# aymenboudhina/Multimodal_VQVAE_compression_audio_tactile

Measured on AMD Instinct MI355X. Metric: encode+VQ+decode token-frames/sec (1 frame = 13.33 ms of paired 24 kHz audio+tactile), higher is better.
Workload: dtype f32

## Files before the change

multimodal_vqvae_compression_audio_tactile_amd/csrc/conv1d_mfma.hpp:

```cpp
#pragma once
#include <hip/hip_runtime.h>
#include <stdio.h>
#include <stdlib.h>
#include <type_traits>
#include "det_math.hpp"
#include "kernels_small.hpp"

namespace mvq {

struct ConvArgs;
inline bool conv_dma_rows_ok(const ConvArgs& a);

__device__ __attribute__((aligned(16))) static const float g_zero16[4] = {0.0f, 0.0f, 0.0f, 0.0f};

int prof_begin(const char* kernel_name, double flops, hipStream_t s);
void prof_end(int idx, hipStream_t s);
bool prof_enabled();

typedef float f32x16 __attribute__((ext_vector_type(16)));
typedef float f32x4 __attribute__((ext_vector_type(4)));

struct ConvArgs {
    const float* x;
    const float* wp;
    const float* bias;
    const float* alpha_in;
    const float* residual;
    const float* alpha_out;
    float* y;
    int B, Cin, Tin, Cout, Tout;
    int pad;
    int Mpad;
    int Mrows;
    int Ncols;
    int n_tiles;
    int n_base;
    int n_tiles_max;
    int row_fast;
    int act;
    int dma;
    int up_s, up_p;
    int vec4;
    int ovec4;
    const float* alpha_mid;
    const float* w2p;
    const float* bias2;
    float* y2;
    const float* alpha2;
    const float* dsn_src;
    const float* dsn_alpha;
    int tvalid;
    int tper, tper_valid;
    unsigned tper_magic;
    int up_per_out, up_valid_out, up_seg, up_btrue;
    unsigned up_magic;
    int vp_seg, vp_per_in, vp_valid_in, vp_tin_phys, vp_btrue, vp_per_out, vp_valid_out;
    unsigned vp_magic_in, vp_magic_out;
    char* name_out;
    int name_len;
};

typedef float f32x16_t __attribute__((ext_vector_type(16)));

template <int OFF>
__device__ __forceinline__ float lds_read_imm(unsigned addr)
{
    static_assert(OFF >= 0 && OFF < 65536, "ds_read immediate offset is 16 bits");
    float v;
    asm volatile("ds_read_b32 %0, %1 offset:%2" : "=v"(v) : "v"(addr), "i"(OFF) : "memory");
    return v;
}
template <int P> __device__ __forceinline__ void lgkm_wait_tie(float& a, float& b)
{ asm volatile("s_waitcnt lgkmcnt(%2)" : "+v"(a), "+v"(b) : "n"(P) : "memory"); }
template <int P> __device__ __forceinline__ void lgkm_wait_tie(float& a, float& b, float& c)
{ asm volatile("s_waitcnt lgkmcnt(%3)" : "+v"(a), "+v"(b), "+v"(c) : "n"(P) : "memory"); }
template <int P> __device__ __forceinline__ void lgkm_wait_tie(float& a, float& b, float& c, float& d)
{ asm volatile("s_waitcnt lgkmcnt(%4)" : "+v"(a), "+v"(b), "+v"(c), "+v"(d) : "n"(P) : "memory"); }
template <int P> __device__ __forceinline__ void lgkm_wait_tie(float& a, float& b, float& c, float& d, float& e)
{ asm volatile("s_waitcnt lgkmcnt(%5)" : "+v"(a), "+v"(b), "+v"(c), "+v"(d), "+v"(e) : "n"(P) : "memory"); }
template <int P> __device__ __forceinline__ void lgkm_wait_tie(float& a, float& b, float& c, float& d, float& e, float& f)
{ asm volatile("s_waitcnt lgkmcnt(%6)" : "+v"(a), "+v"(b), "+v"(c), "+v"(d), "+v"(e), "+v"(f) : "n"(P) : "memory"); }
template <int P, int MT, int NT>
__device__ __forceinline__ void lgkm_wait_step(float (&av)[MT], float (&bv)[NT])
{
    static_assert(MT >= 1 && NT >= 1 && MT + NT <= 6, "operand registers per k-step");
    if constexpr (MT == 1 && NT == 1) lgkm_wait_tie<P>(av[0], bv[0]);
    else if constexpr (MT == 2 && NT == 1) lgkm_wait_tie<P>(av[0], av[1], bv[0]);
    else if constexpr (MT == 1 && NT == 2) lgkm_wait_tie<P>(av[0], bv[0], bv[1]);
    else if constexpr (MT == 2 && NT == 2) lgkm_wait_tie<P>(av[0], av[1], bv[0], bv[1]);
    else if constexpr (MT == 3 && NT == 1) lgkm_wait_tie<P>(av[0], av[1], av[2], bv[0]);
    else if constexpr (MT == 1 && NT == 3) lgkm_wait_tie<P>(av[0], bv[0], bv[1], bv[2]);
    else if constexpr (MT == 4 && NT == 1) lgkm_wait_tie<P>(av[0], av[1], av[2], av[3], bv[0]);
    else if constexpr (MT == 1 && NT == 4) lgkm_wait_tie<P>(av[0], bv[0], bv[1], bv[2], bv[3]);
    else if constexpr (MT == 3 && NT == 2) lgkm_wait_tie<P>(av[0], av[1], av[2], bv[0], bv[1]);
    else if constexpr (MT == 2 && NT == 3) lgkm_wait_tie<P>(av[0], av[1], bv[0], bv[1], bv[2]);
    else if constexpr (MT == 4 && NT == 2) lgkm_wait_tie<P>(av[0], av[1], av[2], av[3], bv[0], bv[1]);
    else if constexpr (MT == 2 && NT == 4) lgkm_wait_tie<P>(av[0], av[1], bv[0], bv[1], bv[2], bv[3]);
    else if constexpr (MT == 3 && NT == 3) lgkm_wait_tie<P>(av[0], av[1], av[2], bv[0], bv[1], bv[2]);
    else static_assert(MT + NT <= 5 || MT == 4 || NT == 4 || (MT == 3 && NT == 3), "unsupported operand shape");
}

#define MVQ_DMA_FIRST(i) "s_nop 0\n\tglobal_load_lds_dwordx4 %" #i ", off\n\t"
#define MVQ_DMA_NEXT(i) "s_add_u32 m0, m0, %[inc]\n\t" MVQ_DMA_FIRST(i)
#define MVQ_DMA_HEAD "s_mov_b32 %0, m0\n\ts_mov_b32 m0, %[dst]\n\t"
#define MVQ_DMA_TAIL "s_mov_b32 m0, %0"
template <int N, int INC>
__device__ __forceinline__ void lds_dma_burst(const float* const* src, unsigned dst)
{
    static_assert(N >= 1 && N <= 8, "pieces per burst");
    unsigned keep;
    if constexpr (N == 1)
        asm volatile(MVQ_DMA_HEAD MVQ_DMA_FIRST(1) MVQ_DMA_TAIL : "=&s"(keep) : "v"(src[0]), [dst] "s"(dst), [inc] "n"(INC) : "memory", "scc");
    else if constexpr (N == 2)
        asm volatile(MVQ_DMA_HEAD MVQ_DMA_FIRST(1) MVQ_DMA_NEXT(2) MVQ_DMA_TAIL
                     : "=&s"(keep) : "v"(src[0]), "v"(src[1]), [dst] "s"(dst), [inc] "n"(INC) : "memory", "scc");
    else if constexpr (N == 3)
        asm volatile(MVQ_DMA_HEAD MVQ_DMA_FIRST(1) MVQ_DMA_NEXT(2) MVQ_DMA_NEXT(3) MVQ_DMA_TAIL
                     : "=&s"(keep) : "v"(src[0]), "v"(src[1]), "v"(src[2]), [dst] "s"(dst), [inc] "n"(INC) : "memory", "scc");
    else if constexpr (N == 4)
        asm volatile(MVQ_DMA_HEAD MVQ_DMA_FIRST(1) MVQ_DMA_NEXT(2) MVQ_DMA_NEXT(3) MVQ_DMA_NEXT(4) MVQ_DMA_TAIL
                     : "=&s"(keep) : "v"(src[0]), "v"(src[1]), "v"(src[2]), "v"(src[3]), [dst] "s"(dst), [inc] "n"(INC) : "memory", "scc");
    else if constexpr (N == 5)
        asm volatile(MVQ_DMA_HEAD MVQ_DMA_FIRST(1) MVQ_DMA_NEXT(2) MVQ_DMA_NEXT(3) MVQ_DMA_NEXT(4) MVQ_DMA_NEXT(5) MVQ_DMA_TAIL
                     : "=&s"(keep) : "v"(src[0]), "v"(src[1]), "v"(src[2]), "v"(src[3]), "v"(src[4]), [dst] "s"(dst), [inc] "n"(INC) : "memory", "scc");
    else if constexpr (N == 6)
        asm volatile(MVQ_DMA_HEAD MVQ_DMA_FIRST(1) MVQ_DMA_NEXT(2) MVQ_DMA_NEXT(3) MVQ_DMA_NEXT(4) MVQ_DMA_NEXT(5) MVQ_DMA_NEXT(6) MVQ_DMA_TAIL
                     : "=&s"(keep) : "v"(src[0]), "v"(src[1]), "v"(src[2]), "v"(src[3]), "v"(src[4]), "v"(src[5]), [dst] "s"(dst), [inc] "n"(INC) : "memory", "scc");
    else if constexpr (N == 7)
        asm volatile(MVQ_DMA_HEAD MVQ_DMA_FIRST(1) MVQ_DMA_NEXT(2) MVQ_DMA_NEXT(3) MVQ_DMA_NEXT(4) MVQ_DMA_NEXT(5) MVQ_DMA_NEXT(6) MVQ_DMA_NEXT(7) MVQ_DMA_TAIL
                     : "=&s"(keep) : "v"(src[0]), "v"(src[1]), "v"(src[2]), "v"(src[3]), "v"(src[4]), "v"(src[5]), "v"(src[6]), [dst] "s"(dst), [inc] "n"(INC) : "memory", "scc");
    else
        asm volatile(MVQ_DMA_HEAD MVQ_DMA_FIRST(1) MVQ_DMA_NEXT(2) MVQ_DMA_NEXT(3) MVQ_DMA_NEXT(4) MVQ_DMA_NEXT(5) MVQ_DMA_NEXT(6) MVQ_DMA_NEXT(7) MVQ_DMA_NEXT(8) MVQ_DMA_TAIL
                     : "=&s"(keep) : "v"(src[0]), "v"(src[1]), "v"(src[2]), "v"(src[3]), "v"(src[4]), "v"(src[5]), "v"(src[6]), "v"(src[7]), [dst] "s"(dst), [inc] "n"(INC) : "memory", "scc");
}

template <int KS, int STRIDE, int DIL, int BM, int XP, int MT, int NT, int NS>
struct AsmOperandLoop {
    template <int S, int I>
    static __device__ __forceinline__ void load_a(float (&av)[MT], unsigned a_addr)
    {
        if constexpr (I < MT) {
            av[I] = lds_read_imm<(2 * S * BM + I * 32) * 4>(a_addr);
            load_a<S, I + 1>(av, a_addr);
        }
    }
    template <int S, int J>
    static __device__ __forceinline__ void load_b(float (&bv)[NT], unsigned b_same, unsigned b_cross)
    {
        if constexpr (J < NT) {
            constexpr int k0 = 2 * S;
            constexpr int off0 = (k0 / KS) * XP + (k0 % KS) * DIL;
            constexpr bool cross = ((k0 + 1) / KS) != (k0 / KS);
            bv[J] = lds_read_imm<(off0 + J * 32 * STRIDE) * 4>(cross ? b_cross : b_same);
            load_b<S, J + 1>(bv, b_same, b_cross);
        }
    }
    template <int S>
    static __device__ __forceinline__ void load_step(float (&av)[MT], float (&bv)[NT], unsigned a_addr, unsigned b_same, unsigned b_cross)
    {
        load_a<S, 0>(av, a_addr);
        load_b<S, 0>(bv, b_same, b_cross);
    }
    static __device__ __forceinline__ void mfma_step(f32x16_t (&acc)[MT][NT], const float (&av)[MT], const float (&bv)[NT])
    {
#pragma unroll
        for (int i = 0; i < MT; ++i)
#pragma unroll
            for (int j = 0; j < NT; ++j)
                acc[i][j] = __builtin_amdgcn_mfma_f32_32x32x2f32(av[i], bv[j], acc[i][j], 0, 0, 0);
    }
    template <int S>
    static __device__ __forceinline__ void run_from(f32x16_t (&acc)[MT][NT], float (&av0)[MT], float (&bv0)[NT], float (&av1)[MT],
                                                    float (&bv1)[NT], unsigned a_addr, unsigned b_same, unsigned b_cross)
    {
        if constexpr (S < NS) {
            if constexpr (S + 1 < NS) {
                if constexpr ((S + 1) % 2 == 0) load_step<S + 1>(av0, bv0, a_addr, b_same, b_cross);
                else load_step<S + 1>(av1, bv1, a_addr, b_same, b_cross);
            }
            constexpr int PW = (S + 1 < NS) ? MT + NT : 0;
            __builtin_amdgcn_sched_barrier(0);
            if constexpr (S % 2 == 0) lgkm_wait_step<PW, MT, NT>(av0, bv0);
            else lgkm_wait_step<PW, MT, NT>(av1, bv1);
            __builtin_amdgcn_sched_barrier(0);
            if constexpr (S % 2 == 0) mfma_step(acc, av0, bv0);
            else mfma_step(acc, av1, bv1);
            __builtin_amdgcn_sched_barrier(0);
            run_from<S + 1>(acc, av0, bv0, av1, bv1, a_addr, b_same, b_cross);
        }
    }
};

constexpr int cgcd(int a, int b) { return b == 0 ? a : cgcd(b, a % b); }

template <int KS, int STRIDE, int DIL, int CK, int MT, int NT, int WAVES_M, int WAVES_N, int UPS>
struct ConvCfg {
    static constexpr int BM = 32 * MT * WAVES_M;
    static constexpr int BN = 32 * NT * WAVES_N;
    static constexpr int KC = CK * KS;
    static constexpr int XT = (BN - 1) * STRIDE + (KS - 1) * DIL + 1;
    static constexpr bool XALIGNED = (KS == 1 && STRIDE == 1);
    static constexpr int XV = XALIGNED ? (XT + 3) / 4 : (XT + 3 + 3) / 4;
    static constexpr int XTP = XV * 4 + 4;
    static constexpr int W_FLOATS = KC * BM;
    static constexpr int X_FLOATS = CK * XTP;
    static constexpr int STAGE_FLOATS = 2 * (W_FLOATS + X_FLOATS);
    static constexpr int BNP = BN + 4;
    static constexpr int CT_FLOATS = BM * BNP;
    static constexpr int EH = ((UPS == 0 || 32 % (UPS ? UPS : 1) == 0) && MT % 2 == 0 && CT_FLOATS > STAGE_FLOATS) ? 2 : 1;
    static constexpr int CTH_FLOATS = CT_FLOATS / EH;
    static constexpr int QPR = BN / 4;
    static constexpr int CQ = cgcd(QPR, 64 * WAVES_M * WAVES_N);
    static constexpr int JN = QPR / CQ;
    static constexpr int RSTEP = (64 * WAVES_M * WAVES_N) / CQ;
    static constexpr bool REG_GEOM = (UPS == 0) && (32 % RSTEP == 0);
    static constexpr int TB_FLOATS = REG_GEOM ? 2 * BM : 0;
    static constexpr int EPI_FLOATS = CTH_FLOATS + TB_FLOATS;
    static constexpr int EPI_FLOATS_FUSE = CT_FLOATS + TB_FLOATS;
    static constexpr int LDS_FLOATS = STAGE_FLOATS > EPI_FLOATS ? STAGE_FLOATS : EPI_FLOATS;
    static constexpr bool FOUR_WAVES = WAVES_M * WAVES_N == 4;
    static constexpr bool RING_FITS = (size_t)3 * (KC * BM + CK * XV * 4) * 4 <= 64 * 1024;
    static constexpr int MIN_WPE = (FOUR_WAVES && LDS_FLOATS * 4 <= 53 * 1024 && !(WAVES_N == 4 && NT == 2) && RING_FITS && MT * NT <= 4) ? 3
                                                                                                                : (WAVES_M * WAVES_N) / 2;
    static constexpr int LDS_FLOATS_FUSE = STAGE_FLOATS > EPI_FLOATS_FUSE ? STAGE_FLOATS : EPI_FLOATS_FUSE;
    static constexpr int MIN_WPE_FUSE = (FOUR_WAVES && (LDS_FLOATS_FUSE + 5 * BM) * 4 * 3 <= 160 * 1024) ? 3 : (WAVES_M * WAVES_N) / 2;
    static constexpr int XV4 = XV * 4;
    static constexpr int DMA_STAGE_FLOATS = W_FLOATS + CK * XV4;
    static constexpr int DMA_NV = DMA_STAGE_FLOATS / 4;
    static constexpr int DMA_NU = (DMA_NV + 64 * WAVES_M * WAVES_N - 1) / (64 * WAVES_M * WAVES_N);
    static constexpr int LDS_FLOATS_DMA = 3 * DMA_STAGE_FLOATS > EPI_FLOATS ? 3 * DMA_STAGE_FLOATS : EPI_FLOATS;
    static constexpr int LDS_FLOATS_FUSE_DMA = 3 * DMA_STAGE_FLOATS > EPI_FLOATS_FUSE ? 3 * DMA_STAGE_FLOATS : EPI_FLOATS_FUSE;
    static constexpr int W_VEC = W_FLOATS / 4;
    static constexpr int NTHR = 64 * WAVES_M * WAVES_N;
    static constexpr int W_PER_THREAD = (W_VEC + NTHR - 1) / NTHR;
    static constexpr int XV_TOTAL = CK * XV;
    static constexpr int XV_PER_THREAD = (XV_TOTAL + NTHR - 1) / NTHR;
    static constexpr int XS_TOTAL = CK * XT;
    static constexpr int XS_PER_THREAD = (XS_TOTAL + NTHR - 1) / NTHR;
    static constexpr int XREGS = (4 * XV_PER_THREAD > XS_PER_THREAD) ? 4 * XV_PER_THREAD : XS_PER_THREAD;
    static_assert(WAVES_M * WAVES_N == 4 || WAVES_M * WAVES_N == 8, "block is 4 or 8 waves");
    static_assert(KC % 2 == 0, "chunk K must be even (32x32x2 MFMA)");
    static_assert(BM % 4 == 0, "float4 weight staging");
};

template <int KS, int STRIDE, int DIL, int CK, int MT, int NT, int WAVES_M, int WAVES_N, int UPS, bool VEC>
struct ConvTile {
    using C = ConvCfg<KS, STRIDE, DIL, CK, MT, NT, WAVES_M, WAVES_N, UPS>;
    const float* wp; const float* xb; const float* Al;
    float* Ws; float* Xs;
    int tid, Tin, Cin, Mpad, m0, t_in0, g_al;
    bool snake_in;

    __device__ __forceinline__ void load_chunk(int chunk, f32x4 (&wreg)[C::W_PER_THREAD], f32x4 (&xv)[C::XV_PER_THREAD], float (&xs)[C::XS_PER_THREAD]) const
    {
        const int ci0 = chunk * CK;
        const float* wsrc = wp + (size_t)ci0 * KS * Mpad + m0;
#pragma unroll
        for (int u = 0; u < C::W_PER_THREAD; ++u) {
            int v = tid + u * C::NTHR;
            if (C::W_VEC % C::NTHR != 0) v = v < C::W_VEC ? v : C::W_VEC - 1;
            const int row = v / (C::BM / 4);
            const int c4 = v - row * (C::BM / 4);
            wreg[u] = *reinterpret_cast<const f32x4*>(wsrc + (size_t)row * Mpad + c4 * 4);
        }
        if (VEC) {
#pragma unroll
            for (int u = 0; u < C::XV_PER_THREAD; ++u) {
                int e = tid + u * C::NTHR;
                if (C::XV_TOTAL % C::NTHR != 0) e = e < C::XV_TOTAL ? e : C::XV_TOTAL - 1;
                const int cl = e / C::XV;
                const int v = e - cl * C::XV;
                const int g = g_al + 4 * v;
                const bool ok = g >= 0 && g < Tin;
                const int gc = ok ? g : 0;
                xv[u] = *reinterpret_cast<const f32x4*>(xb + (size_t)(ci0 + cl) * Tin + gc);
            }
        } else {
#pragma unroll
            for (int u = 0; u < C::XS_PER_THREAD; ++u) {
                int e = tid + u * C::NTHR;
                if (C::XS_TOTAL % C::NTHR != 0) e = e < C::XS_TOTAL ? e : C::XS_TOTAL - 1;
                const int cl = e / C::XT;
                const int xi = e - cl * C::XT;
                const int g = t_in0 + xi;
                const bool ok = g >= 0 && g < Tin;
                const int gc = ok ? g : 0;
                xs[u] = xb[(size_t)(ci0 + cl) * Tin + gc];
            }
        }
    }

    __device__ __forceinline__ void store_chunk(int chunk, int buf, const f32x4 (&wreg)[C::W_PER_THREAD],
                                                const f32x4 (&xv)[C::XV_PER_THREAD],
                                                const float (&xs)[C::XS_PER_THREAD]) const
    {
        const int ci0 = chunk * CK;
        float* wdst = Ws + buf * C::W_FLOATS;
        float* xdst = Xs + buf * C::X_FLOATS;
#pragma unroll
        for (int u = 0; u < C::W_PER_THREAD; ++u) {
            const int v = tid + u * C::NTHR;
            if (C::W_VEC % C::NTHR == 0 || v < C::W_VEC) *reinterpret_cast<f32x4*>(wdst + v * 4) = wreg[u];
        }
        if (VEC) {
#pragma unroll
            for (int u = 0; u < C::XV_PER_THREAD; ++u) {
                const int e = tid + u * C::NTHR;
                const int ec = (C::XV_TOTAL % C::NTHR != 0 && e >= C::XV_TOTAL) ? C::XV_TOTAL - 1 : e;
                const int cl = ec / C::XV;
                const int v = ec - cl * C::XV;
                const int g = g_al + 4 * v;
                const bool ok = g >= 0 && g < Tin;
                f32x4 q = xv[u];
                if (!ok) q = f32x4{0.0f, 0.0f, 0.0f, 0.0f};
                if (snake_in) {
                    const float al = Al[ci0 + cl], inv = Al[Cin + ci0 + cl];
                    q.x = det_snake(q.x, al, inv); q.y = det_snake(q.y, al, inv);
                    q.z = det_snake(q.z, al, inv); q.w = det_snake(q.w, al, inv);
                }
                if (C::XV_TOTAL % C::NTHR == 0 || e < C::XV_TOTAL)
                    *reinterpret_cast<f32x4*>(xdst + cl * C::XTP + 4 * v) = q;
            }
        } else {
#pragma unroll
            for (int u = 0; u < C::XS_PER_THREAD; ++u) {
                const int e = tid + u * C::NTHR;
                const int ec = (C::XS_TOTAL % C::NTHR != 0 && e >= C::XS_TOTAL) ? C::XS_TOTAL - 1 : e;
                const int cl = ec / C::XT;
                const int xi = ec - cl * C::XT;
                const int g = t_in0 + xi;
                float q = (g >= 0 && g < Tin) ? xs[u] : 0.0f;
                if (snake_in) q = det_snake(q, Al[ci0 + cl], Al[Cin + ci0 + cl]);
                if (C::XS_TOTAL % C::NTHR == 0 || e < C::XS_TOTAL) xdst[cl * C::XTP + xi] = q;
            }
        }
    }
};

template <int KS, int STRIDE, int DIL, int CK, int MT, int NT, int WAVES_M, int WAVES_N, int UPS, bool VEC, bool FUSE>
__device__ __forceinline__ void conv1d_mfma_body(const ConvArgs& a)
{
    using C = ConvCfg<KS, STRIDE, DIL, CK, MT, NT, WAVES_M, WAVES_N, UPS>;
    extern __shared__ __attribute__((aligned(16))) float smem[];
    float* const Ws = smem;
    float* const Xs = smem + 2 * C::W_FLOATS;
    float* const Ep = smem + (FUSE ? (a.dma ? C::LDS_FLOATS_FUSE_DMA : C::LDS_FLOATS_FUSE) : (a.dma ? C::LDS_FLOATS_DMA : C::LDS_FLOATS));
    constexpr int EP_MID = 2;
    float* const Al = Ep + 3 * C::BM;

    const int tid = threadIdx.x;
    const int lane = tid & 63;
    const int wave = tid >> 6;
    const int wm = wave / WAVES_N;
    const int wn = wave % WAVES_N;
    const int l31 = lane & 31;
    const int h = lane >> 5;

    int bx = blockIdx.x, by = blockIdx.y;
    if (a.row_fast) {
        const int xcd = bx & 7, j = bx >> 3;
        by = j % a.row_fast;
        bx = (j / a.row_fast) * 8 + xcd;
        if (bx >= a.n_tiles * a.B) return;
    }
    const int b = bx / a.n_tiles;
    const int tile_n = bx - b * a.n_tiles;
    const int n0 = a.n_base + tile_n * C::BN;
    const int m0 = by * C::BM;
    const int t_in0 = n0 * STRIDE - a.pad;
    const int g_al = t_in0 & ~3;
    const int shift = VEC ? (t_in0 - g_al) : 0;
    const int Cin = a.Cin;
    const int n_chunks = Cin / CK;
    const bool snake_in = a.alpha_in != nullptr;

    if (snake_in) {
        for (int c = tid; c < Cin; c += C::NTHR) {
            const float al = a.alpha_in[c];
            Al[c] = al;
            Al[Cin + c] = 1.0f / (al + 1e-9f);
        }
    }
    for (int r = tid; r < C::BM; r += C::NTHR) {
        int m = m0 + r;
        m = m < a.Mrows ? m : a.Mrows - 1;
        const int ch = m / (UPS ? UPS : 1);
        const float* tabs[4] = {a.alpha_out, a.y2 ? a.alpha2 : nullptr, FUSE ? a.alpha_mid : (a.dsn_src ? a.dsn_alpha : nullptr), nullptr};
#pragma unroll
        for (int k = 0; k < 3; ++k) {
            Ep[k * C::BM + r] = tabs[k] ? 1.0f / (tabs[k][ch] + 1e-9f) : 1.0f;
        }
    }

    ConvTile<KS, STRIDE, DIL, CK, MT, NT, WAVES_M, WAVES_N, UPS, VEC> tile;
    tile.wp = a.wp; tile.xb = a.x + (size_t)b * Cin * a.Tin; tile.Al = Al; tile.Ws = Ws; tile.Xs = Xs;
    tile.tid = tid; tile.Tin = a.Tin; tile.Cin = Cin; tile.Mpad = a.Mpad; tile.m0 = m0; tile.t_in0 = t_in0;
    tile.g_al = g_al; tile.snake_in = snake_in;

    f32x16 acc[MT][NT];
#pragma unroll
    for (int i = 0; i < MT; ++i)
#pragma unroll
        for (int j = 0; j < NT; ++j)
#pragma unroll
            for (int r = 0; r < 16; ++r) acc[i][j][r] = 0.0f;

    f32x4 wreg[C::W_PER_THREAD];
    f32x4 xv[C::XV_PER_THREAD];
    float xs[C::XS_PER_THREAD];

    constexpr int D_SAME = DIL;
    constexpr int D_CROSS = C::XTP - (KS - 1) * DIL;
    const int a_base = h * C::BM + wm * (MT * 32) + l31;
    const int b_base = (wn * (NT * 32) + l31) * STRIDE + shift;
    const int b_same = b_base + h * D_SAME;
    const int b_cross = b_base + h * D_CROSS;

    constexpr int NS = C::KC / 2;
    auto mfma_chunk = [&](int buf) __attribute__((always_inline)) {
        const float* wsrc = Ws + buf * C::W_FLOATS + a_base;
        const float* xs_same = Xs + buf * C::X_FLOATS + b_same;
        const float* xs_cross = Xs + buf * C::X_FLOATS + b_cross;
        float av[2][MT], bv[2][NT];
        auto load_step = [&](int st, int pb) __attribute__((always_inline)) {
            const int k0 = 2 * st;
            const int off0 = (k0 / KS) * C::XTP + (k0 % KS) * DIL;
            const bool cross = ((k0 + 1) / KS) != (k0 / KS);
            const float* xsp = cross ? xs_cross : xs_same;
#pragma unroll
            for (int i = 0; i < MT; ++i) av[pb][i] = wsrc[k0 * C::BM + i * 32];
#pragma unroll
            for (int j = 0; j < NT; ++j) bv[pb][j] = xsp[off0 + j * 32 * STRIDE];
        };
        load_step(0, 0);
#pragma unroll
        for (int s = 0; s < NS; ++s) {
            const int pb = s & 1;
            if (s + 1 < NS) load_step(s + 1, (s + 1) & 1);
#pragma unroll
            for (int i = 0; i < MT; ++i)
#pragma unroll
                for (int j = 0; j < NT; ++j)
                    acc[i][j] = __builtin_amdgcn_mfma_f32_32x32x2f32(av[pb][i], bv[pb][j], acc[i][j], 0, 0, 0);
            __builtin_amdgcn_sched_group_barrier(0x100, MT + NT, 0);
            __builtin_amdgcn_sched_group_barrier(0x008, MT * NT, 0);
        }
    };

    constexpr bool DMA_FITS = FUSE ? ((size_t)C::LDS_FLOATS_FUSE_DMA + 3 * C::BM) * 4 * 2 <= 160 * 1024 : (size_t)C::LDS_FLOATS_DMA * 4 <= 64 * 1024;
    bool use_dma = false;
    if constexpr (VEC && DMA_FITS) use_dma = a.dma != 0;
    if (use_dma) {
      if constexpr (VEC && DMA_FITS) {
        constexpr int NU = C::DMA_NU;
        constexpr int XP = C::XV4;
        constexpr int D_CROSS_D = XP - (KS - 1) * DIL;
        const int bd_same = b_base + h * D_SAME;
        const int bd_cross = b_base + h * D_CROSS_D;
        const float* src[NU];
        bool live[NU];
        long long step_b[NU];
#pragma unroll
        for (int u = 0; u < NU; ++u) {
            const int p = tid + u * C::NTHR;
            live[u] = p < C::DMA_NV;
            if (p < C::W_VEC) {
                const int row = p / (C::BM / 4), c4 = p - row * (C::BM / 4);
                src[u] = a.wp + (size_t)row * a.Mpad + m0 + c4 * 4;
                step_b[u] = (long long)CK * KS * a.Mpad;
            } else {
                const int q = (p < C::DMA_NV ? p : C::DMA_NV - 1) - C::W_VEC;
                const int cl = q / C::XV, v = q - cl * C::XV;
                const int g = g_al + 4 * v;
                bool ok = g >= 0 && g < a.Tin;
                const float* sp = tile.xb + (size_t)cl * a.Tin + g;
                long long st = (long long)CK * a.Tin;
                if (a.vp_seg) {
                    const int gg = ok ? g : 0;
                    const int seg = (int)__umulhi((unsigned)gg, a.vp_magic_in), pos = gg - seg * a.vp_per_in;
                    const int item = b * a.vp_seg + seg;
                    ok = ok && pos < a.vp_valid_in && item < a.vp_btrue;
                    sp = a.x + ((size_t)(ok ? item : 0) * a.Cin + cl) * a.vp_tin_phys + (ok ? pos : 0);
                    st = (long long)CK * a.vp_tin_phys;
                }
                src[u] = ok ? sp : g_zero16;
                step_b[u] = ok ? st : 0;
            }
        }
        const unsigned lds0 = (unsigned)(size_t)smem;
        const int wave_u = __builtin_amdgcn_readfirstlane(wave);
        const int n_issue = (NU - 1) * C::NTHR + wave_u * 64 < C::DMA_NV ? NU : NU - 1;
        constexpr int NFULL = C::DMA_NV / C::NTHR < NU ? C::DMA_NV / C::NTHR : NU;
        auto dma_chunk = [&](int stage) __attribute__((always_inline)) {
            const unsigned dst0 = lds0 + (unsigned)(stage * C::DMA_STAGE_FLOATS * 4) + (unsigned)(wave_u * 64 * 16);
            if constexpr (NFULL > 0) lds_dma_burst<NFULL, C::NTHR * 16>(src, dst0);
#pragma unroll
            for (int u = NFULL; u < NU; ++u) {
                if (live[u]) lds_dma_burst<1, C::NTHR * 16>(src + u, dst0 + (unsigned)(u * C::NTHR * 16));
            }
#pragma unroll
            for (int u = 0; u < NU; ++u) src[u] += step_b[u];
        };
        using AL = AsmOperandLoop<KS, STRIDE, DIL, C::BM, XP, MT, NT, NS>;
        auto mfma_chunk_asm = [&](int stage, bool issue_next, int next_stage) __attribute__((always_inline)) {
            const unsigned sb = lds0 + (unsigned)(stage * C::DMA_STAGE_FLOATS * 4);
            const unsigned a_addr = sb + (unsigned)(a_base * 4);
            const unsigned b_s = sb + (unsigned)((C::W_FLOATS + bd_same) * 4), b_c = sb + (unsigned)((C::W_FLOATS + bd_cross) * 4);
            float av0[MT], bv0[NT], av1[MT], bv1[NT];
            AL::template load_step<0>(av0, bv0, a_addr, b_s, b_c);
            if (issue_next) dma_chunk(next_stage);
            AL::template run_from<0>(acc, av0, bv0, av1, bv1, a_addr, b_s, b_c);
        };
        dma_chunk(0);
        if (n_chunks > 1) dma_chunk(1);
        int st_c = 0, st_n2 = 2;
        for (int c = 0; c < n_chunks; ++c) {
            if (c + 1 >= n_chunks) asm volatile("s_waitcnt vmcnt(0)" ::: "memory");
            else if (n_issue == NU) asm volatile("s_waitcnt vmcnt(%0)" :: "n"(NU) : "memory");
            else asm volatile("s_waitcnt vmcnt(%0)" :: "n"(NU - 1) : "memory");
            __syncthreads();
            mfma_chunk_asm(st_c, c + 2 < n_chunks, st_n2);
            st_c = st_c == 2 ? 0 : st_c + 1;
            st_n2 = st_n2 == 2 ? 0 : st_n2 + 1;
        }
      }
    } else {
    tile.load_chunk(0, wreg, xv, xs);
    __syncthreads();
    tile.store_chunk(0, 0, wreg, xv, xs);
    __syncthreads();
    for (int c = 0; c + 1 < n_chunks; ++c) {
        tile.load_chunk(c + 1, wreg, xv, xs);
        __builtin_amdgcn_sched_barrier(0);
        mfma_chunk(c & 1);
        __builtin_amdgcn_sched_barrier(0);
        tile.store_chunk(c + 1, (c + 1) & 1, wreg, xv, xs);
        __syncthreads();
    }
    mfma_chunk((n_chunks - 1) & 1);
    }

    const float* ep_bias = a.bias;
    if (FUSE) {
        float* const Ht = smem;
        __syncthreads();
#pragma unroll
        for (int i = 0; i < MT; ++i)
#pragma unroll
            for (int r = 0; r < 16; ++r) {
                const int row = (wm * MT + i) * 32 + (r & 3) + 8 * (r >> 2) + 4 * h;
                const float bv = a.bias ? a.bias[row] : 0.0f;
                const float al = a.alpha_mid[row], inv = Ep[EP_MID * C::BM + row];
#pragma unroll
                for (int j = 0; j < NT; ++j) {
                    Ht[row * C::BNP + (wn * NT + j) * 32 + l31] = det_snake(acc[i][j][r] + bv, al, inv);
                    acc[i][j][r] = 0.0f;
                }
            }
        __syncthreads();
        constexpr int K2 = C::BM / 2;
        constexpr int G = 8;
        static_assert(K2 % G == 0, "BM must be a multiple of 16");
        const float* w2 = a.w2p + (size_t)h * a.Mpad + wm * (MT * 32) + l31;
        const float* hsrc = Ht + h * C::BNP + wn * (NT * 32) + l31;
        float aw[2][G][MT];
#pragma unroll
        for (int g = 0; g < G; ++g)
#pragma unroll
            for (int i = 0; i < MT; ++i) aw[0][g][i] = w2[(size_t)(2 * g) * a.Mpad + i * 32];
#pragma unroll
        for (int grp = 0; grp < K2 / G; ++grp) {
            if (grp + 1 < K2 / G) {
#pragma unroll
                for (int g = 0; g < G; ++g)
#pragma unroll
                    for (int i = 0; i < MT; ++i)
                        aw[(grp + 1) & 1][g][i] = w2[(size_t)(2 * ((grp + 1) * G + g)) * a.Mpad + i * 32];
            }
#pragma unroll
            for (int g = 0; g < G; ++g) {
                const int s2 = grp * G + g;
                float bvv[NT];
#pragma unroll
                for (int j = 0; j < NT; ++j) bvv[j] = hsrc[2 * s2 * C::BNP + j * 32];
#pragma unroll
                for (int i = 0; i < MT; ++i)
#pragma unroll
                    for (int j = 0; j < NT; ++j)
                        acc[i][j] = __builtin_amdgcn_mfma_f32_32x32x2f32(aw[grp & 1][g][i], bvv[j], acc[i][j], 0, 0, 0);
            }
        }
        ep_bias = a.bias2;
    }

    const bool has_res = (UPS == 0) && a.residual != nullptr;
    const bool snake_out = a.alpha_out != nullptr;
    const bool do_tanh = a.act == 1;
    const bool do_gelu = a.act == 2;
    const bool direct = (UPS != 0) && (C::BM % (UPS ? UPS : 1) != 0);
    if (direct) {
#pragma unroll
        for (int i = 0; i < MT; ++i) {
#pragma unroll
            for (int r = 0; r < 16; ++r) {
                const int row = (r & 3) + 8 * (r >> 2) + 4 * h;
                const int m = m0 + (wm * MT + i) * 32 + row;
                const bool mok = m < a.Mrows;
                const int mc = mok ? m : a.Mrows - 1;
                const int co = mc / (UPS ? UPS : 1), rr = mc - co * (UPS ? UPS : 1);
                const float bv = ep_bias ? ep_bias[co] : 0.0f;
                const int lr = (wm * MT + i) * 32 + row;
                const float al = snake_out ? a.alpha_out[co] : 1.0f, inv = Ep[lr];
                const size_t rowoff = ((size_t)b * a.Cout + co) * a.Tout;
#pragma unroll
                for (int j = 0; j < NT; ++j) {
                    const int n = n0 + (wn * NT + j) * 32 + l31;
                    int t = n * (UPS ? UPS : 1) + rr - a.up_p;
                    bool ok = mok && n < a.Ncols && t >= 0 && (a.up_per_out ? true : t < a.Tout);
                    t = ok ? t : 0;
                    size_t ro = rowoff;
                    if (a.up_per_out) {
                        const int sg = (int)__umulhi((unsigned)t, a.up_magic);
                        t -= sg * a.up_per_out;
                        const int bb = b * a.up_seg + sg;
                        ok = ok && t < a.up_valid_out && bb < a.up_btrue;
                        ro = ((size_t)(ok ? bb : 0) * a.Cout + co) * a.Tout;
                        t = ok ? t : 0;
                    }
                    float v = acc[i][j][r] + bv;
                    const bool tail = a.tvalid && t >= a.tvalid;
                    if (ok && a.y2) a.y2[ro + t] = tail ? 0.0f : det_snake(v, a.alpha2[co], Ep[C::BM + lr]);
                    if (snake_out) v = det_snake(v, al, inv);
                    if (ok) a.y[ro + t] = tail ? 0.0f : v;
                }
            }
        }
        return;
    }

    float* const Ct = smem;
    constexpr int EHP = FUSE ? 1 : C::EH;
    constexpr int MTH = MT / EHP;
    constexpr int BMH = C::BM / EHP;
    auto tile_row_of = [&](int lrow, int pass) __attribute__((always_inline)) {
        if (EHP == 1) return lrow;
        const int g = lrow >> 5;
        return ((g / MTH) * MT + pass * MTH + (g % MTH)) * 32 + (lrow & 31);
    };
    auto epilogue_pass = [&](auto HP) __attribute__((always_inline)) {
    constexpr int hp = decltype(HP)::value;
    __syncthreads();
#pragma unroll
    for (int il = 0; il < MTH; ++il)
#pragma unroll
        for (int r = 0; r < 16; ++r) {
            const int row = (wm * MTH + il) * 32 + (r & 3) + 8 * (r >> 2) + 4 * h;
#pragma unroll
            for (int j = 0; j < NT; ++j) Ct[row * C::BNP + (wn * NT + j) * 32 + l31] = acc[hp * MTH + il][j][r];
        }
    constexpr int NVQ = BMH * C::BN / 4;
    constexpr bool PRE_RES = (UPS == 0) && (NVQ % C::NTHR == 0) && (NVQ / C::NTHR <= 16);
    constexpr int RES_IT = PRE_RES ? NVQ / C::NTHR : 1;
    constexpr int CQ = C::CQ, JN = C::JN;
    constexpr bool REG = PRE_RES && C::REG_GEOM && (BMH % C::RSTEP == 0);
    constexpr int RSTEP = REG ? C::RSTEP : 1;
    const bool reg_ok = REG && !(a.y2 && a.alpha_out);
    const int q_c0 = REG ? tid % CQ : 0, q_r0 = REG ? tid / CQ : 0;
    auto reg_k = [&](int it, int pass) __attribute__((always_inline)) {
        const int lr = (it / JN) * RSTEP;
        if (EHP == 1) return lr;
        const int g = lr >> 5;
        return ((g / MTH) * MT + pass * MTH + (g % MTH)) * 32 + (lr & 31);
    };
    const size_t blk_off = a.vp_seg ? ((size_t)b * a.vp_seg * a.Cout + m0) * a.Tout : ((size_t)b * a.Cout + m0) * a.Tout + n0;
    const unsigned q_t0 = (unsigned)(q_r0 * a.Tout);
    bool q_nok[JN];
    unsigned q_col[JN];
    int q_vpos[JN];
#pragma unroll
    for (int j = 0; j < JN; ++j) {
        const int n = n0 + 4 * (q_c0 + j * CQ);
        q_nok[j] = n < a.Ncols;
        q_col[j] = 4u * (q_c0 + j * CQ);
        q_vpos[j] = 0;
        if (a.vp_seg) {
            const int nn = q_nok[j] ? n : 0;
            const int seg = (int)__umulhi((unsigned)nn, a.vp_magic_out), pos = nn - seg * a.vp_per_out;
            q_nok[j] = q_nok[j] && b * a.vp_seg + seg < a.vp_btrue && pos < a.Tout;
            q_col[j] = (unsigned)(seg * a.Cout * a.Tout + pos);
            q_vpos[j] = pos;
        }
    }
    f32x4 res_q[RES_IT];
    if (PRE_RES && has_res && a.ovec4) {
        bool pre_done = false;
        if constexpr (REG) if (reg_ok) {
            pre_done = true;
            const float* resb = a.residual + blk_off;
#pragma unroll
            for (int it = 0; it < RES_IT; ++it) {
                const int k = reg_k(it, hp), j = it % JN;
                const bool ok = q_nok[j] && m0 + q_r0 + k < a.Mrows;
                res_q[it] = *reinterpret_cast<const f32x4*>(resb + (ok ? q_t0 + (unsigned)(k * a.Tout) + q_col[j] : 0u));
            }
        }
        if (!pre_done) {
#pragma unroll
            for (int it = 0; it < RES_IT; ++it) {
                const int e = tid + it * C::NTHR;
                const int row = e / (C::BN / 4);
                const int c4 = e - row * (C::BN / 4);
                const int m = m0 + tile_row_of(row, hp), n = n0 + 4 * c4;
                const bool ok = m < a.Mrows && n < a.Ncols;
                const size_t off = ((size_t)b * a.Cout + (ok ? m : 0)) * a.Tout + (ok ? n : 0);
                res_q[it] = *reinterpret_cast<const f32x4*>(a.residual + off);
            }
        }
    }
    float* const Tb = smem + (FUSE ? C::CT_FLOATS : C::CTH_FLOATS);
    if (reg_ok && hp == 0) {
        const float* const ax = a.y2 ? a.alpha2 : a.alpha_out;
        for (int r = tid; r < C::BM; r += C::NTHR) {
            int m = m0 + r;
            m = m < a.Mrows ? m : a.Mrows - 1;
            Tb[r] = ep_bias ? ep_bias[m] : 0.0f;
            Tb[C::BM + r] = ax ? ax[m] : 1.0f;
        }
    }
    __syncthreads();
    auto tile_row = [&](int lrow) __attribute__((always_inline)) { return tile_row_of(lrow, hp); };

    if (UPS == 0) {
        if (a.ovec4) {
            constexpr int NV = BMH * C::BN / 4;
            auto quad = [&](int e, int it) __attribute__((always_inline)) {
                const int row = e / (C::BN / 4);
                const int c4 = e - row * (C::BN / 4);
                const int m = m0 + tile_row(row), n = n0 + 4 * c4;
                if (m < a.Mrows && n < a.Ncols) {
                    const float bv = ep_bias ? ep_bias[m] : 0.0f;
                    f32x4 v = *reinterpret_cast<const f32x4*>(Ct + row * C::BNP + 4 * c4);
                    const size_t off = ((size_t)b * a.Cout + m) * a.Tout + n;
                    v.x = v.x + bv; v.y = v.y + bv; v.z = v.z + bv; v.w = v.w + bv;
                    if (a.dsn_src) {
                        const float ad = a.dsn_alpha[m], id = Ep[2 * C::BM + tile_row(row)];
                        const f32x4 sv = *reinterpret_cast<const f32x4*>(a.dsn_src + off);
                        v.x = v.x * det_dsnake(sv.x, ad, id); v.y = v.y * det_dsnake(sv.y, ad, id);
                        v.z = v.z * det_dsnake(sv.z, ad, id); v.w = v.w * det_dsnake(sv.w, ad, id);
                    }
                    if (has_res) {
                        const f32x4 rv = PRE_RES ? res_q[PRE_RES ? it : 0] : *reinterpret_cast<const f32x4*>(a.residual + off);
                        v.x = v.x + rv.x; v.y = v.y + rv.y; v.z = v.z + rv.z; v.w = v.w + rv.w;
                    }
                    int nz = (a.tvalid && n + 4 > a.tvalid) ? n + 4 - a.tvalid : 0;
                    if (a.tper) {
                        const int nn = n - (int)__umulhi((unsigned)n, a.tper_magic) * a.tper;
                        nz = nn + 4 > a.tper_valid ? (nn >= a.tper_valid ? 4 : nn + 4 - a.tper_valid) : 0;
                    }
                    if (a.y2) {
                        const float a2 = a.alpha2[m], i2 = Ep[C::BM + tile_row(row)];
                        f32x4 w = {det_snake(v.x, a2, i2), det_snake(v.y, a2, i2), det_snake(v.z, a2, i2), det_snake(v.w, a2, i2)};
                        if (nz > 0) { w.w = 0.0f; if (nz > 1) w.z = 0.0f; if (nz > 2) w.y = 0.0f; if (nz > 3) w.x = 0.0f; }
                        *reinterpret_cast<f32x4*>(a.y2 + off) = w;
                    }
                    if (snake_out) {
                        const float al = a.alpha_out[m], inv = Ep[tile_row(row)];
                        v.x = det_snake(v.x, al, inv); v.y = det_snake(v.y, al, inv);
                        v.z = det_snake(v.z, al, inv); v.w = det_snake(v.w, al, inv);
                    }
                    if (do_tanh) { v.x = det_tanh(v.x); v.y = det_tanh(v.y); v.z = det_tanh(v.z); v.w = det_tanh(v.w); }
                    if (do_gelu) { v.x = det_gelu(v.x); v.y = det_gelu(v.y); v.z = det_gelu(v.z); v.w = det_gelu(v.w); }
                    if (nz > 0) { v.w = 0.0f; if (nz > 1) v.z = 0.0f; if (nz > 2) v.y = 0.0f; if (nz > 3) v.x = 0.0f; }
                    *reinterpret_cast<f32x4*>(a.y + off) = v;
                }
            };
            bool quads_done = false;
            if constexpr (REG) if (reg_ok) {
                quads_done = true;
                int nz[JN];
#pragma unroll
                for (int j = 0; j < JN; ++j) {
                    const int n = n0 + 4 * (q_c0 + j * CQ);
                    nz[j] = (a.tvalid && n + 4 > a.tvalid) ? n + 4 - a.tvalid : 0;
                    if (a.tper) {
                        const int nn = n - (int)__umulhi((unsigned)n, a.tper_magic) * a.tper;
                        nz[j] = nn + 4 > a.tper_valid ? (nn >= a.tper_valid ? 4 : nn + 4 - a.tper_valid) : 0;
                    }
                    if (a.vp_seg) {
                        const int pp = q_vpos[j];
                        nz[j] = pp + 4 > a.vp_valid_out ? (pp >= a.vp_valid_out ? 4 : pp + 4 - a.vp_valid_out) : 0;
                    }
                }
                float* const yb = a.y + blk_off;
                float* const y2b = a.y2 ? a.y2 + blk_off : nullptr;
                const float* const dsb = a.dsn_src ? a.dsn_src + blk_off : nullptr;
                const float* const ctq = Ct + q_r0 * C::BNP + 4 * q_c0;
                const float* const tbq = Tb + q_r0;
                const float* const epq = Ep + q_r0;
                auto reg_quads = [&](auto MODE_) __attribute__((always_inline)) {
                    constexpr int MODE = decltype(MODE_)::value;
                    const bool f_dsn = MODE == 0 ? (a.dsn_src != nullptr) : false;
                    const bool f_res = MODE == 0 ? has_res : (MODE == 1 || MODE == 2 || MODE == 5);
                    const bool f_y2 = MODE == 0 ? (a.y2 != nullptr) : (MODE == 1 || MODE == 4);
                    const bool f_so = MODE == 0 ? snake_out : (MODE == 2 || MODE == 3);
                    const bool f_tanh = MODE == 0 ? do_tanh : false;
                    const bool f_gelu = MODE == 0 ? do_gelu : false;
#pragma unroll
                    for (int it = 0; it < RES_IT; ++it) {
                        const int k = reg_k(it, hp), j = it % JN;
                        const int trow = q_r0 + k;
                        if (q_nok[j] && m0 + trow < a.Mrows) {
                            const unsigned toff = q_t0 + (unsigned)(k * a.Tout) + q_col[j];
                            const float bv = tbq[k];
                            f32x4 v = *reinterpret_cast<const f32x4*>(ctq + (it / JN) * RSTEP * C::BNP + 4 * CQ * j);
                            v.x = v.x + bv; v.y = v.y + bv; v.z = v.z + bv; v.w = v.w + bv;
                            if (f_dsn) {
                                const float ad = a.dsn_alpha[m0 + trow], id = epq[2 * C::BM + k];
                                const f32x4 sv = *reinterpret_cast<const f32x4*>(dsb + toff);
                                v.x = v.x * det_dsnake(sv.x, ad, id); v.y = v.y * det_dsnake(sv.y, ad, id);
                                v.z = v.z * det_dsnake(sv.z, ad, id); v.w = v.w * det_dsnake(sv.w, ad, id);
                            }
                            if (f_res) {
                                const f32x4 rv = res_q[it];
                                v.x = v.x + rv.x; v.y = v.y + rv.y; v.z = v.z + rv.z; v.w = v.w + rv.w;
                            }
                            const int z = nz[j];
// ... 331 lines not shown
```

Baseline: 60650.

## Add uniform-base LDS DMA path with scalar bases and unrolled triple-buffer loop

Result: faster. 61560, median of 6 (+1.5%).

```diff
diff --git a/multimodal_vqvae_compression_audio_tactile_amd/csrc/conv1d_mfma.hpp b/multimodal_vqvae_compression_audio_tactile_amd/csrc/conv1d_mfma.hpp
--- a/multimodal_vqvae_compression_audio_tactile_amd/csrc/conv1d_mfma.hpp
+++ b/multimodal_vqvae_compression_audio_tactile_amd/csrc/conv1d_mfma.hpp
@@ -134,13 +134,63 @@
                      : "=&s"(keep) : "v"(src[0]), "v"(src[1]), "v"(src[2]), "v"(src[3]), "v"(src[4]), "v"(src[5]), "v"(src[6]), "v"(src[7]), [dst] "s"(dst), [inc] "n"(INC) : "memory", "scc");
 }
 
-template <int KS, int STRIDE, int DIL, int BM, int XP, int MT, int NT, int NS>
+#define MVQ_DMAU_FIRST(i) "s_nop 0\n\tglobal_load_lds_dwordx4 %" #i ", %[base]\n\t"
+#define MVQ_DMAU_NEXT(i) "s_add_u32 m0, m0, %[inc]\n\t" MVQ_DMAU_FIRST(i)
+template <int N, int INC>
+__device__ __forceinline__ void lds_dma_burst_uni(const unsigned* off, unsigned long long base, unsigned dst)
+{
+    static_assert(N >= 1 && N <= 8, "pieces per burst");
+    unsigned keep;
+    if constexpr (N == 1)
+        asm volatile(MVQ_DMA_HEAD MVQ_DMAU_FIRST(1) MVQ_DMA_TAIL : "=&s"(keep) : "v"(off[0]), [base] "s"(base), [dst] "s"(dst), [inc] "n"(INC) : "memory", "scc");
+    else if constexpr (N == 2)
+        asm volatile(MVQ_DMA_HEAD MVQ_DMAU_FIRST(1) MVQ_DMAU_NEXT(2) MVQ_DMA_TAIL
+                     : "=&s"(keep) : "v"(off[0]), "v"(off[1]), [base] "s"(base), [dst] "s"(dst), [inc] "n"(INC) : "memory", "scc");
+    else if constexpr (N == 3)
+        asm volatile(MVQ_DMA_HEAD MVQ_DMAU_FIRST(1) MVQ_DMAU_NEXT(2) MVQ_DMAU_NEXT(3) MVQ_DMA_TAIL
+                     : "=&s"(keep) : "v"(off[0]), "v"(off[1]), "v"(off[2]), [base] "s"(base), [dst] "s"(dst), [inc] "n"(INC) : "memory", "scc");
+    else if constexpr (N == 4)
+        asm volatile(MVQ_DMA_HEAD MVQ_DMAU_FIRST(1) MVQ_DMAU_NEXT(2) MVQ_DMAU_NEXT(3) MVQ_DMAU_NEXT(4) MVQ_DMA_TAIL
+                     : "=&s"(keep) : "v"(off[0]), "v"(off[1]), "v"(off[2]), "v"(off[3]), [base] "s"(base), [dst] "s"(dst), [inc] "n"(INC) : "memory", "scc");
+    else if constexpr (N == 5)
+        asm volatile(MVQ_DMA_HEAD MVQ_DMAU_FIRST(1) MVQ_DMAU_NEXT(2) MVQ_DMAU_NEXT(3) MVQ_DMAU_NEXT(4) MVQ_DMAU_NEXT(5) MVQ_DMA_TAIL
+                     : "=&s"(keep) : "v"(off[0]), "v"(off[1]), "v"(off[2]), "v"(off[3]), "v"(off[4]), [base] "s"(base), [dst] "s"(dst), [inc] "n"(INC) : "memory", "scc");
+    else if constexpr (N == 6)
+        asm volatile(MVQ_DMA_HEAD MVQ_DMAU_FIRST(1) MVQ_DMAU_NEXT(2) MVQ_DMAU_NEXT(3) MVQ_DMAU_NEXT(4) MVQ_DMAU_NEXT(5) MVQ_DMAU_NEXT(6) MVQ_DMA_TAIL
+                     : "=&s"(keep) : "v"(off[0]), "v"(off[1]), "v"(off[2]), "v"(off[3]), "v"(off[4]), "v"(off[5]), [base] "s"(base), [dst] "s"(dst), [inc] "n"(INC) : "memory", "scc");
+    else if constexpr (N == 7)
+        asm volatile(MVQ_DMA_HEAD MVQ_DMAU_FIRST(1) MVQ_DMAU_NEXT(2) MVQ_DMAU_NEXT(3) MVQ_DMAU_NEXT(4) MVQ_DMAU_NEXT(5) MVQ_DMAU_NEXT(6) MVQ_DMAU_NEXT(7) MVQ_DMA_TAIL
+                     : "=&s"(keep) : "v"(off[0]), "v"(off[1]), "v"(off[2]), "v"(off[3]), "v"(off[4]), "v"(off[5]), "v"(off[6]), [base] "s"(base), [dst] "s"(dst), [inc] "n"(INC) : "memory", "scc");
+    else
+        asm volatile(MVQ_DMA_HEAD MVQ_DMAU_FIRST(1) MVQ_DMAU_NEXT(2) MVQ_DMAU_NEXT(3) MVQ_DMAU_NEXT(4) MVQ_DMAU_NEXT(5) MVQ_DMAU_NEXT(6) MVQ_DMAU_NEXT(7) MVQ_DMAU_NEXT(8) MVQ_DMA_TAIL
+                     : "=&s"(keep) : "v"(off[0]), "v"(off[1]), "v"(off[2]), "v"(off[3]), "v"(off[4]), "v"(off[5]), "v"(off[6]), "v"(off[7]), [base] "s"(base), [dst] "s"(dst), [inc] "n"(INC) : "memory", "scc");
+}
+__device__ __forceinline__ void lds_dma_masked_uni(unsigned off, unsigned long long base, unsigned dst, unsigned long long mask)
+{
+    unsigned keep;
+    unsigned long long keep_exec;
+    asm volatile("s_mov_b64 %1, exec\n\ts_mov_b64 exec, %[mask]\n\t"
+                 "s_mov_b32 %0, m0\n\ts_mov_b32 m0, %[dst]\n\ts_nop 0\n\tglobal_load_lds_dwordx4 %2, %[base]\n\ts_mov_b32 m0, %0\n\t"
+                 "s_mov_b64 exec, %1"
+                 : "=&s"(keep), "=&s"(keep_exec) : "v"(off), [base] "s"(base), [dst] "s"(dst), [mask] "s"(mask) : "memory");
+}
+
+__device__ __forceinline__ unsigned long long dma_scalar_base(const float* p)
+{
+    const unsigned long long v = (unsigned long long)p;
+    const unsigned lo = __builtin_amdgcn_readfirstlane((unsigned)v), hi = __builtin_amdgcn_readfirstlane((unsigned)(v >> 32));
+    unsigned long long s = ((unsigned long long)hi << 32) | lo;
+    asm volatile("s_nop 4" : "+s"(s));
+    return s;
+}
+
+template <int KS, int STRIDE, int DIL, int BM, int XP, int MT, int NT, int NS, int BASE = 0>
 struct AsmOperandLoop {
     template <int S, int I>
     static __device__ __forceinline__ void load_a(float (&av)[MT], unsigned a_addr)
     {
         if constexpr (I < MT) {
-            av[I] = lds_read_imm<(2 * S * BM + I * 32) * 4>(a_addr);
+            av[I] = lds_read_imm<BASE + (2 * S * BM + I * 32) * 4>(a_addr);
             load_a<S, I + 1>(av, a_addr);
         }
     }
@@ -151,7 +201,7 @@
             constexpr int k0 = 2 * S;
             constexpr int off0 = (k0 / KS) * XP + (k0 % KS) * DIL;
             constexpr bool cross = ((k0 + 1) / KS) != (k0 / KS);
-            bv[J] = lds_read_imm<(off0 + J * 32 * STRIDE) * 4>(cross ? b_cross : b_same);
+            bv[J] = lds_read_imm<BASE + (off0 + J * 32 * STRIDE) * 4>(cross ? b_cross : b_same);
             load_b<S, J + 1>(bv, b_same, b_cross);
         }
     }
@@ -457,6 +507,103 @@
         constexpr int D_CROSS_D = XP - (KS - 1) * DIL;
         const int bd_same = b_base + h * D_SAME;
         const int bd_cross = b_base + h * D_CROSS_D;
+        const unsigned lds0 = (unsigned)(size_t)smem;
+        const int wave_u = __builtin_amdgcn_readfirstlane(wave);
+        using AL = AsmOperandLoop<KS, STRIDE, DIL, C::BM, XP, MT, NT, NS>;
+        auto chunk_rt = [&](int stage, auto&& issue) __attribute__((always_inline)) {
+            const unsigned sb = lds0 + (unsigned)(stage * C::DMA_STAGE_FLOATS * 4);
+            const unsigned a_addr = sb + (unsigned)(a_base * 4);
+            const unsigned b_s = sb + (unsigned)((C::W_FLOATS + bd_same) * 4), b_c = sb + (unsigned)((C::W_FLOATS + bd_cross) * 4);
+            float av0[MT], bv0[NT], av1[MT], bv1[NT];
+            AL::template load_step<0>(av0, bv0, a_addr, b_s, b_c);
+            issue();
+            AL::template run_from<0>(acc, av0, bv0, av1, bv1, a_addr, b_s, b_c);
+        };
+        constexpr int NW = WAVES_M * WAVES_N;
+        constexpr int XPC = CK * C::XV;
+        constexpr int WI_W = (C::W_VEC + 63) / 64, WI_X = (XPC + 63) / 64;
+        constexpr int NU_W = (WI_W + NW - 1) / NW, NU_X = (WI_X + NW - 1) / NW;
+        constexpr int NF_W = C::W_VEC / C::NTHR, NF_X = XPC / C::NTHR;
+        static_assert(NU_W - NF_W <= 1 && NU_X - NF_X <= 1, "at most one masked instruction per kind");
+        constexpr int NI_MIN = (WI_W + WI_X) / NW;
+        constexpr bool UNI_OK = (size_t)3 * C::DMA_STAGE_FLOATS * 4 <= 65536 && NF_W <= 8 && NF_X <= 8;
+        bool uni = false;
+        if constexpr (UNI_OK) uni = !a.vp_seg && g_al >= 0 && g_al + 4 * C::XV <= a.Tin && (long long)CK * a.Tin < (1ll << 29);
+        if (uni) {
+          if constexpr (UNI_OK) {
+            unsigned woff[NU_W], xoff[NU_X];
+#pragma unroll
+            for (int u = 0; u < NU_W; ++u) {
+                int p = tid + u * C::NTHR;
+                p = p < C::W_VEC ? p : C::W_VEC - 1;
+                const int row = p / (C::BM / 4), c4 = p - row * (C::BM / 4);
+                woff[u] = (unsigned)(row * a.Mpad + c4 * 4) * 4u;
+            }
+            const int xw = (wave_u + NW - WI_W % NW) % NW;
+#pragma unroll
+            for (int j = 0; j < NU_X; ++j) {
+                int q = (xw + j * NW) * 64 + lane;
+                q = q < XPC ? q : XPC - 1;
+                const int cl = q / C::XV, v = q - cl * C::XV;
+                xoff[j] = (unsigned)(cl * a.Tin + 4 * v) * 4u;
+            }
+            unsigned long long mask_w = 0, mask_x = 0;
+            if constexpr (NU_W > NF_W) mask_w = __ballot(tid + NF_W * C::NTHR < C::W_VEC);
+            if constexpr (NU_X > NF_X) mask_x = __ballot((xw + NF_X * NW) * 64 + lane < XPC);
+            unsigned long long wbase = dma_scalar_base(a.wp + m0);
+            unsigned long long xbase = dma_scalar_base(tile.xb + g_al);
+            const unsigned wstep = (unsigned)(CK * KS * a.Mpad) * 4u, xstep = (unsigned)(CK * a.Tin) * 4u;
+            const unsigned wdst0 = lds0 + (unsigned)(wave_u * 1024), xdst0 = lds0 + (unsigned)(C::W_FLOATS * 4) + (unsigned)(xw * 1024);
+            auto dma_uni = [&](int stage) __attribute__((always_inline)) {
+                const unsigned so = (unsigned)(stage * C::DMA_STAGE_FLOATS * 4);
+                if constexpr (NF_W > 0) lds_dma_burst_uni<NF_W, C::NTHR * 16>(woff, wbase, wdst0 + so);
+                if constexpr (NU_W > NF_W) lds_dma_masked_uni(woff[NU_W - 1], wbase, wdst0 + so + (unsigned)(NF_W * C::NTHR * 16), mask_w);
+                if constexpr (NF_X > 0) lds_dma_burst_uni<NF_X, C::NTHR * 16>(xoff, xbase, xdst0 + so);
+                if constexpr (NU_X > NF_X) lds_dma_masked_uni(xoff[NU_X - 1], xbase, xdst0 + so + (unsigned)(NF_X * C::NTHR * 16), mask_x);
+                wbase += wstep;
+                xbase += xstep;
+            };
+            const unsigned a_addr0 = lds0 + (unsigned)(a_base * 4);
+            const unsigned b_s0 = lds0 + (unsigned)((C::W_FLOATS + bd_same) * 4), b_c0 = lds0 + (unsigned)((C::W_FLOATS + bd_cross) * 4);
+            auto chunk_uni = [&](auto STAGE_) __attribute__((always_inline)) {
+                constexpr int STAGE = decltype(STAGE_)::value;
+                using ALS = AsmOperandLoop<KS, STRIDE, DIL, C::BM, XP, MT, NT, NS, STAGE * C::DMA_STAGE_FLOATS * 4>;
+                float av0[MT], bv0[NT], av1[MT], bv1[NT];
+                ALS::template load_step<0>(av0, bv0, a_addr0, b_s0, b_c0);
+                dma_uni((STAGE + 2) % 3);
+                ALS::template run_from<0>(acc, av0, bv0, av1, bv1, a_addr0, b_s0, b_c0);
+            };
+            auto k_loop_uni = [&](auto NWAIT_) __attribute__((always_inline)) {
+                constexpr int NWAIT = decltype(NWAIT_)::value;
+                int c = 0;
+                for (; c + 5 <= n_chunks; c += 3) {
+                    asm volatile("s_waitcnt vmcnt(%0)" :: "n"(NWAIT) : "memory");
+                    __syncthreads();
+                    chunk_uni(std::integral_constant<int, 0>{});
+                    asm volatile("s_waitcnt vmcnt(%0)" :: "n"(NWAIT) : "memory");
+                    __syncthreads();
+                    chunk_uni(std::integral_constant<int, 1>{});
+                    asm volatile("s_waitcnt vmcnt(%0)" :: "n"(NWAIT) : "memory");
+                    __syncthreads();
+                    chunk_uni(std::integral_constant<int, 2>{});
+                }
+                int st_c = 0, st_n2 = 2;
+                for (; c < n_chunks; ++c) {
+                    if (c + 1 >= n_chunks) asm volatile("s_waitcnt vmcnt(0)" ::: "memory");
+                    else asm volatile("s_waitcnt vmcnt(%0)" :: "n"(NWAIT) : "memory");
+                    __syncthreads();
+                    chunk_rt(st_c, [&]() __attribute__((always_inline)) { if (c + 2 < n_chunks) dma_uni(st_n2); });
+                    st_c = st_c == 2 ? 0 : st_c + 1;
+                    st_n2 = st_n2 == 2 ? 0 : st_n2 + 1;
+                }
+            };
+            dma_uni(0);
+            if (n_chunks > 1) dma_uni(1);
+            const int my_issue = (WI_W - wave_u + NW - 1) / NW + (WI_X - xw + NW - 1) / NW;
+            if ((WI_W + WI_X) % NW != 0 && my_issue > NI_MIN) k_loop_uni(std::integral_constant<int, NI_MIN + 1>{});
+            else k_loop_uni(std::integral_constant<int, NI_MIN>{});
+          }
+        } else {
         const float* src[NU];
         bool live[NU];
         long long step_b[NU];
@@ -487,8 +634,6 @@
                 step_b[u] = ok ? st : 0;
             }
         }
-        const unsigned lds0 = (unsigned)(size_t)smem;
-        const int wave_u = __builtin_amdgcn_readfirstlane(wave);
         const int n_issue = (NU - 1) * C::NTHR + wave_u * 64 < C::DMA_NV ? NU : NU - 1;
         constexpr int NFULL = C::DMA_NV / C::NTHR < NU ? C::DMA_NV / C::NTHR : NU;
         auto dma_chunk = [&](int stage) __attribute__((always_inline)) {
@@ -500,16 +645,6 @@
             }
 #pragma unroll
             for (int u = 0; u < NU; ++u) src[u] += step_b[u];
-        };
-        using AL = AsmOperandLoop<KS, STRIDE, DIL, C::BM, XP, MT, NT, NS>;
-        auto mfma_chunk_asm = [&](int stage, bool issue_next, int next_stage) __attribute__((always_inline)) {
-            const unsigned sb = lds0 + (unsigned)(stage * C::DMA_STAGE_FLOATS * 4);
-            const unsigned a_addr = sb + (unsigned)(a_base * 4);
-            const unsigned b_s = sb + (unsigned)((C::W_FLOATS + bd_same) * 4), b_c = sb + (unsigned)((C::W_FLOATS + bd_cross) * 4);
-            float av0[MT], bv0[NT], av1[MT], bv1[NT];
-            AL::template load_step<0>(av0, bv0, a_addr, b_s, b_c);
-            if (issue_next) dma_chunk(next_stage);
-            AL::template run_from<0>(acc, av0, bv0, av1, bv1, a_addr, b_s, b_c);
         };
         dma_chunk(0);
         if (n_chunks > 1) dma_chunk(1);
@@ -519,9 +654,10 @@
             else if (n_issue == NU) asm volatile("s_waitcnt vmcnt(%0)" :: "n"(NU) : "memory");
             else asm volatile("s_waitcnt vmcnt(%0)" :: "n"(NU - 1) : "memory");
             __syncthreads();
-            mfma_chunk_asm(st_c, c + 2 < n_chunks, st_n2);
+            chunk_rt(st_c, [&]() __attribute__((always_inline)) { if (c + 2 < n_chunks) dma_chunk(st_n2); });
             st_c = st_c == 2 ? 0 : st_c + 1;
             st_n2 = st_n2 == 2 ? 0 : st_n2 + 1;
+        }
         }
       }
     } else {
```
